# vineetbansal/scarlet

Hardware: AMD Instinct MI355X
Metric: PGM iters/sec on 10k 5-band 64x64 scenes (higher is better)
Workload: dtype f32

## Files before the change

scarlet_amd/csrc/fused2.h:

```cpp
#pragma once
#include "fused.h"

#define SC_FB2 512
#define SC_NW2 (SC_FB2 / SC_WAVE)
#define SC_PAIR_VEC_FLOATS 512

struct KsLengths {
    unsigned short v[2][32];
    static constexpr int fast_len(int n)
    {
        for (int m = n;; ++m) {
            int q = m;
            while (q % 2 == 0) q /= 2;
            while (q % 3 == 0) q /= 3;
            while (q % 5 == 0) q /= 5;
            if (q == 1) return m;
        }
    }
    constexpr KsLengths() : v{}
    {
        for (int r = 0; r < 32; ++r) {
            const int F = fast_len(2 * (2 * r + 1) + 10);
            int Fe = F;
            while (Fe & 1) Fe = fast_len(Fe + 1);
            v[0][r] = (unsigned short)F; v[1][r] = (unsigned short)Fe;
        }
    }
};
__device__ const KsLengths sc_ks_lengths = KsLengths();
__device__ __forceinline__ unsigned ks_request_lengths(int tid)
{
    return tid < 64 ? (unsigned)(&sc_ks_lengths.v[0][0])[tid] : 0u;
}
__device__ __forceinline__ void ks_fill_lengths(unsigned short (*fl)[32], int tid, unsigned requested)
{
    if (tid < 64) (&fl[0][0])[tid] = (unsigned short)requested;
}
__device__ __forceinline__ KsGeom ks_geom(const SymWindow &s, const unsigned short (*fl)[32])
{
    KsGeom g;
    g.h = s.h; g.w = s.w; g.ry = s.h / 2; g.rx = s.w / 2;
    g.ntr = round16(s.h) >> 4; g.wp = round16(s.w); g.ntc = g.wp >> 4;
    g.Fy = uniform((int)fl[0][g.ry]);
    g.Fx = uniform((int)fl[1][g.rx]);
    return g;
}

template <int KM, int BM, int XS, bool P>
__device__ __forceinline__ int iterate2_body(const FusedArgs &a, const int s, const int c0, const int it_old, const bool resident,
                                             const bool reentered = false)
{
    static_assert(KM <= 4, "one pair of waves per component");
    static_assert(1 + KM * BM <= 32 && 4 * SC_NW2 == 32, "the partial sums are combined by 32 rows of 16 lanes");
    constexpr bool X = XS > 0;
    extern __shared__ __align__(16) float lds[];
    const int K = X ? KM : a.K, B = X ? BM : a.B, H = X ? XS : a.H, W = X ? XS : a.W, HW = H * W, LW = X ? SC_XS_STRIDE : tile_stride(W);
    const int tile_floats = H * LW;
#ifndef SC_TILE_B128
#define SC_TILE_B128 1
#endif
    auto tl4 = [](const float *p) {
        if constexpr (X && SC_TILE_B128 && (SC_XS_STRIDE % 4) == 0) return *reinterpret_cast<const float4 *>(p);
        else return lds_load4(p);
    };
    auto ts4 = [](float *p, float4 v) {
        if constexpr (X && SC_TILE_B128 && (SC_XS_STRIDE % 4) == 0) *reinterpret_cast<float4 *>(p) = v;
        else lds_store4(p, v);
    };
    const bool symmetric = X ? true : a.symmetric != 0, monotonic = X ? true : a.monotonic != 0;
    float *tiles = lds;
    float *vecs = lds + (size_t)K * tile_floats;
    constexpr int NG = KM * (KM + 1) / 2;
    constexpr int NP = 1 + KM * BM;
    constexpr int GPT = 2;
    constexpr int GPW = 8;
    __shared__ float red[4 * SC_NW2][NP > NG ? NP : NG];
    __shared__ double mat[2][KM * KM > BM * BM ? KM * KM : BM * BM];
    __shared__ float sed_s[KM * BM], sed_new[KM * BM];
    __shared__ float step_s[2];
    __shared__ double conv_s[KM][2], conv_m[KM][2][2];
    __shared__ int lstop_s[KM];
    __shared__ float nmax_s[KM][2];
    __shared__ int pair_flag[KM][2];
    __shared__ double cent_s[KM][2][3];
    __shared__ unsigned short fl_s[2][32];
    __shared__ int ctl_s[2][2];
    __shared__ int carry_cen[KM][2];
    __shared__ double carry_sh[KM][2];
    __shared__ float carry_sed[KM * BM];
    __shared__ short rowrange_s[KM][2][2];
    const int tid = threadIdx.x, lane = tid & 63, wid = uniform(tid >> 6);
    float *const morph0 = a.morph[0], *const morph1 = a.morph[1], *const sed0 = a.sed[0], *const sed1 = a.sed[1];
    const float *min_g = (c0 ? morph1 : morph0) + (size_t)s * K * HW;
    float *mout_g = (c0 ? morph0 : morph1) + (size_t)s * K * HW;
    const float *sed_in = (c0 ? sed1 : sed0) + (size_t)s * K * B;
    float *sed_out = (c0 ? sed0 : sed1) + (size_t)s * K * B;
    const int it_new = it_old + 1;
    const int ngroups = HW >> 2, gpr = W >> 2;
    const float *img = a.images + (size_t)s * B * HW;
    const float *wgt = (!X && a.weights) ? a.weights + (size_t)s * B * HW : nullptr;
#define STAMP(i) do { if (a.stamps && tid == 0) a.stamps[(size_t)s * 16 + (i)] = (long long)__builtin_amdgcn_s_memtime(); } while (0)
    STAMP(0);
    if (a.stamps && tid == 0) a.stamps[(size_t)s * 16 + 7] = (long long)__builtin_amdgcn_s_memrealtime();
#ifdef SC_STAMP_PERIOD
    if (P && a.stamps && tid == 0) a.stamps[(size_t)a.S * 16 + (size_t)s * 2 + (it_new & 1)] = (long long)__builtin_amdgcn_s_memrealtime();
#endif
    if (P && a.stamps && tid == 0 && !reentered) {
        a.stamps[(size_t)s * 16 + 14] = (long long)__builtin_amdgcn_s_memrealtime();
        a.stamps[(size_t)s * 16 + 15] = (long long)__builtin_amdgcn_s_getreg(4 | (0 << 6) | (31 << 11))
                                        | ((long long)__builtin_amdgcn_s_getreg(20 | (0 << 6) | (31 << 11)) << 32);
    }
    const unsigned fl_req = ks_request_lengths(tid);
    int pre_cy = 0, pre_cx = 0;
    double pre_dy = 0, pre_dx = 0;
    if (X && (wid >> 1) < K) {
        const int cpre = s * K + (wid >> 1);
        if (!(P && reentered)) {
            pre_cy = a.centers[2 * cpre]; pre_cx = a.centers[2 * cpre + 1];
            pre_dy = a.shifts[2 * cpre]; pre_dx = a.shifts[2 * cpre + 1];
        }
        if (P) {
            const int lcy = carry_cen[wid >> 1][0], lcx = carry_cen[wid >> 1][1];
            const double ldy = carry_sh[wid >> 1][0], ldx = carry_sh[wid >> 1][1];
            if (reentered) { pre_cy = lcy; pre_cx = lcx; pre_dy = ldy; pre_dx = ldx; }
        }
    }
    float *kcache = nullptr;
    float kc_v[3] = {0.f, 0.f, 0.f};
    unsigned kc_hdr = 0;
    if (X && a.kscache && (wid >> 1) < K) {
        kcache = a.kscache + ((size_t)(s * K + (wid >> 1)) * 2 + (wid & 1)) * SC_KSC_FLOATS;
        if (P) {
            kc_v[0] = __builtin_nontemporal_load(kcache + lane); kc_v[1] = __builtin_nontemporal_load(kcache + 64 + lane);
            kc_v[2] = __builtin_nontemporal_load(kcache + 128 + lane);
            kc_hdr = __builtin_nontemporal_load(reinterpret_cast<const unsigned *>(kcache) + 192 + (lane & 7));
        } else {
            kc_v[0] = kcache[lane]; kc_v[1] = kcache[64 + lane]; kc_v[2] = kcache[128 + lane];
            kc_hdr = reinterpret_cast<const unsigned *>(kcache)[192 + (lane & 7)];
        }
    }

    float4 mreg[GPT][KM];
    auto load4 = [&](const float *p, bool past_l1) {
        if (P && past_l1) {
            const f32x4 v = __builtin_nontemporal_load(reinterpret_cast<const f32x4 *>(p));
            return make_float4(v[0], v[1], v[2], v[3]);
        }
        return *reinterpret_cast<const float4 *>(p);
    };
    if (!P || !resident) {
#pragma unroll
        for (int j = 0; j < GPT; ++j) {
            const int g = tid + j * SC_FB2;
#pragma unroll
            for (int k = 0; k < KM; ++k)
                mreg[j][k] = (g < ngroups && k < K) ? load4(min_g + (size_t)k * HW + 4 * (size_t)g, reentered)
                                                   : make_float4(0.f, 0.f, 0.f, 0.f);
        }
    }
    float4 ireg[GPT][BM];
    auto load_images = [&](int j) {
        const int g = tid + j * SC_FB2;
#pragma unroll
        for (int b = 0; b < BM; ++b)
            ireg[j][b] = (g < ngroups && b < B) ? reinterpret_cast<const float4 *>(img + (size_t)b * HW)[g]
                                               : make_float4(0.f, 0.f, 0.f, 0.f);
    };
    load_images(0);
    for (int i = tid; i < K * B; i += SC_FB2) {
        float v = 0.f;
        if (!(P && reentered)) v = sed_in[i];
        if (P) { const float lv = carry_sed[(i / B) * BM + (i % B)]; if (reentered) v = lv; }
        if (P && !reentered) carry_sed[(i / B) * BM + (i % B)] = v;
        sed_s[(i / B) * BM + (i % B)] = v;
    }
    ks_fill_lengths(fl_s, tid, fl_req);
    if (tid < 2 * KM) (&pair_flag[0][0])[tid] = 0;
    if (P && tid == 0) { ctl_s[it_old & 1][0] = 1; ctl_s[it_old & 1][1] = 1; }
    if (P && !reentered && tid < KM * 4) (&rowrange_s[0][0][0])[tid] = (short)((tid & 1) ? H - 1 : 0);
    if (P && resident) {
#pragma unroll
        for (int j = 0; j < GPT; ++j) {
            const int g = tid + j * SC_FB2;
            const int y = g / gpr, x = (g - y * gpr) << 2;
#pragma unroll
            for (int k = 0; k < KM; ++k)
                mreg[j][k] = (g < ngroups && k < K) ? tl4(tiles + k * tile_floats + y * LW + x) : make_float4(0.f, 0.f, 0.f, 0.f);
        }
    }
    const bool small_side = (K <= B);
    __syncthreads();
    {
        f32x2 gram2[NG];
#pragma unroll
        for (int i = 0; i < NG; ++i) gram2[i] = (f32x2){0.f, 0.f};
#pragma unroll
        for (int j = 0; j < GPT; ++j) {
            const int g = tid + j * SC_FB2;
            if (g < ngroups) {
                const int y = g / gpr, x = (g - y * gpr) << 2;
#pragma unroll
                for (int k = 0; k < KM; ++k)
                    if (k < K && !(P && resident)) ts4(tiles + k * tile_floats + y * LW + x, mreg[j][k]);
                int gi = 0;
#pragma unroll
                for (int k = 0; k < KM; ++k)
#pragma unroll
                    for (int k2 = k; k2 < KM; ++k2) {
                        const float4 p = mreg[j][k], q = mreg[j][k2];
                        gram2[gi] += (f32x2){p.x, p.y} * (f32x2){q.x, q.y};
                        gram2[gi] += (f32x2){p.z, p.w} * (f32x2){q.z, q.w};
                        ++gi;
                    }
            }
        }
        float gram[NG];
#pragma unroll
        for (int i = 0; i < NG; ++i) gram[i] = gram2[i].x + gram2[i].y;
        float gq[(NG + 3) / 4];
        wave_rowsum_quads(gram, gq);
        if ((lane & 12) == 12) {
#pragma unroll
            for (int m = 0; m < (NG + 3) / 4; ++m)
                if (4 * m + 3 < NG || 4 * m + (lane & 3) < NG) red[4 * wid + (lane >> 4)][4 * m + (lane & 3)] = gq[m];
        }
    }
#pragma unroll
    for (int j = 1; j < GPT; ++j) load_images(j);
    __syncthreads();
    STAMP(1);
    if (wid == 0) {
        {
            const int e = lane >> 2, q = lane & 3;
            const int k = e / K, k2 = e - k * K;
            const int lo = k < k2 ? k : k2, hi = k < k2 ? k2 : k;
            const int go = lo * KM - (lo * (lo - 1)) / 2 + (hi - lo);
            double r = 0;
            if (e < K * K) {
#pragma unroll
                for (int w = 0; w < SC_NW2; ++w) r += (double)red[q * SC_NW2 + w][go];
            }
            r += dpp_mov<SC_DPP_XOR1>(r);
            r += dpp_mov<SC_DPP_XOR2>(r);
            if (e < K * K && q == 0) mat[0][k * KM + k2] = r;
        }
        if (lane < (small_side ? K * K : B * B)) {
            double r = 0;
            if (small_side) {
                const int k = lane / K, k2 = lane - k * K;
                for (int b = 0; b < B; ++b) r += (double)sed_s[k * BM + b] * sed_s[k2 * BM + b];
                mat[1][k * KM + k2] = r;
            } else {
                const int b = lane / B, b2 = lane - b * B;
                for (int k = 0; k < K; ++k) r += (double)sed_s[k * BM + b] * sed_s[k * BM + b2];
                mat[1][b * BM + b2] = r;
            }
        }
        wave_sync();
        if (lane < 2) {
            const int n = (lane == 0 || small_side) ? K : B, ld = (lane == 0 || small_side) ? KM : BM;
            const double L = n <= 4 ? lambda_max_charpoly4(mat[lane], n, ld) : jacobi_lambda_max(mat[lane], n, ld);
            step_s[lane] = 1.0f / (float)L;
            a.lipschitz[2 * s + lane] = L;
        }
    }
    __syncthreads();
    STAMP(2);
    const float step_sed = step_s[0], step_morph = step_s[1];

    {
        float sed[KM][BM];
#pragma unroll
        for (int k = 0; k < KM; ++k)
#pragma unroll
            for (int b = 0; b < BM; ++b)
                sed[k][b] = (k < K && b < B) ? __builtin_bit_cast(float, __builtin_amdgcn_readfirstlane(
                                                   __builtin_bit_cast(int, sed_s[k * BM + b]))) : 0.f;
        bool fixm[KM];
#pragma unroll
        for (int k = 0; k < KM; ++k) fixm[k] = (k < K) && a.fix_morph && a.fix_morph[(size_t)s * K + k];
        f32x2 dsed2[KM][BM];
#pragma unroll
        for (int k = 0; k < KM; ++k)
#pragma unroll
            for (int b = 0; b < BM; ++b) dsed2[k][b] = (f32x2){0.f, 0.f};
        f32x2 loss2 = {0.f, 0.f};
        const f32x2 ws2 = {a.weight_scalar, a.weight_scalar};
#pragma unroll
        for (int j = 0; j < GPT; ++j) {
            const int g = tid + j * SC_FB2;
            if (g < ngroups) {
                const int y = g / gpr, x = (g - y * gpr) << 2;
                f32x2 m2[KM][2], gm2[KM][2];
#pragma unroll
                for (int k = 0; k < KM; ++k) {
                    float4 v = make_float4(0.f, 0.f, 0.f, 0.f);
                    if (k < K) v = tl4(tiles + k * tile_floats + y * LW + x);
                    m2[k][0] = (f32x2){v.x, v.y}; m2[k][1] = (f32x2){v.z, v.w};
                    gm2[k][0] = (f32x2){0.f, 0.f}; gm2[k][1] = gm2[k][0];
                }
#pragma unroll
                for (int b = 0; b < BM; ++b) {
                    if (b < B) {
                        const float4 iv = ireg[j][b];
                        f32x2 im2[2] = {{iv.x, iv.y}, {iv.z, iv.w}}, ww2[2] = {ws2, ws2};
                        if (wgt) {
                            const float4 wv = reinterpret_cast<const float4 *>(wgt + (size_t)b * HW)[g];
                            ww2[0] = (f32x2){wv.x, wv.y}; ww2[1] = (f32x2){wv.z, wv.w};
                        }
#pragma unroll
                        for (int p = 0; p < 2; ++p) {
                            f32x2 model = sed[0][b] * m2[0][p];
#pragma unroll
                            for (int k = 1; k < KM; ++k) model += sed[k][b] * m2[k][p];
                            const f32x2 d = X ? model - im2[p] : ww2[p] * (model - im2[p]);
                            loss2 = (f32x2){__builtin_fmaf(d.x, d.x, loss2.x), __builtin_fmaf(d.y, d.y, loss2.y)};
                            const f32x2 gg = X ? d : ww2[p] * d;
#pragma unroll
                            for (int k = 0; k < KM; ++k) { dsed2[k][b] += gg * m2[k][p]; gm2[k][p] += sed[k][b] * gg; }
                        }
                    }
                }
#pragma unroll
                for (int k = 0; k < KM; ++k)
                    if (k < K && !fixm[k]) {
                        const f32x2 o0 = m2[k][0] - step_morph * gm2[k][0], o1 = m2[k][1] - step_morph * gm2[k][1];
                        ts4(tiles + k * tile_floats + y * LW + x, make_float4(o0.x, o0.y, o1.x, o1.y));
                    }
            }
        }
        float part[NP];
        part[0] = 0.5f * (loss2.x + loss2.y);
#pragma unroll
        for (int k = 0; k < KM; ++k)
#pragma unroll
            for (int b = 0; b < BM; ++b) part[1 + k * BM + b] = dsed2[k][b].x + dsed2[k][b].y;
        float pq[(NP + 3) / 4];
        wave_rowsum_quads(part, pq);
        if ((lane & 12) == 12) {
#pragma unroll
            for (int m = 0; m < (NP + 3) / 4; ++m)
                if (4 * m + 3 < NP || 4 * m + (lane & 3) < NP) red[4 * wid + (lane >> 4)][4 * m + (lane & 3)] = pq[m];
        }
    }
    __syncthreads();
    STAMP(3);
    {
        const int i = tid >> 4, p = tid & 15;
        const bool live = i < 1 + K * B;
        const int src = (!live || i == 0) ? 0 : 1 + ((i - 1) / B) * BM + (i - 1) % B;
        double r = live ? (double)red[p][src] + (double)red[p + 16][src] : 0.0;
        r += dpp_mov<SC_DPP_XOR1>(r);
        r += dpp_mov<SC_DPP_XOR2>(r);
        r += dpp_mov<SC_DPP_HALF_MIRROR>(r);
        r += dpp_mov<SC_DPP_MIRROR>(r);
        if (live && p == 0) {
            if (i == 0) {
                if (it_new <= a.mse_capacity) a.mse[(size_t)s * a.mse_capacity + it_new - 1] = r;
            } else {
                const int k = (i - 1) / B, b = (i - 1) - k * B;
                const float curv = sed_s[k * BM + b];
                const bool fixed = a.fix_sed && a.fix_sed[(size_t)s * K + k];
                sed_new[k * BM + b] = fixed ? curv : curv - step_sed * (float)r;
            }
        }
    }
    __syncthreads();
    STAMP(4);

    const int k = wid >> 1, half = wid & 1;
    const bool lead = half == ((k >> 1) & 1);
    auto pair_sync = [&](int phase, auto long_wait) {
        constexpr bool LONG = decltype(long_wait)::value;
        __builtin_amdgcn_fence(__ATOMIC_RELEASE, "workgroup");
        if (lane == 0) __hip_atomic_store(&pair_flag[k & (KM - 1)][half], phase, __ATOMIC_RELAXED, __HIP_MEMORY_SCOPE_WORKGROUP);
        while (__hip_atomic_load(&pair_flag[k & (KM - 1)][1 - half], __ATOMIC_RELAXED, __HIP_MEMORY_SCOPE_WORKGROUP) < phase) {
            if (LONG) __builtin_amdgcn_s_sleep(8); else __builtin_amdgcn_s_sleep(2);
        }
        __builtin_amdgcn_fence(__ATOMIC_ACQUIRE, "workgroup");
    };
    const int n_present = a.ncomp ? scene_ncomp(a.ncomp, s, K) : K;
    const bool mine = k < n_present;
    const int c = s * K + (mine ? k : 0);
    Tile t; t.H = H; t.W = W; t.LW = LW; t.m = tiles + (mine ? k : 0) * tile_floats;
    float *vec = vecs + (mine ? k : 0) * SC_PAIR_VEC_FLOATS;
    float *zv = vec + 384 + SC_WAVE * half;
    int cy = 0, cx = 0, stat = 0;
    int mode = 0;
    SymWindow sw = {0, 0, 1, 1, true};
    KsGeom kg = {};
    float sy = 0.f;
    bool rank1 = false;
    if (mine) {
        cy = X ? pre_cy : a.centers[2 * c]; cx = X ? pre_cx : a.centers[2 * c + 1];
        wave_max_pixel(t, cy, cx, stat);
        cy = uniform(cy); cx = uniform(cx);
        if (symmetric) {
            double dy = X ? pre_dy : a.shifts[2 * c], dx = X ? pre_dx : a.shifts[2 * c + 1];
            if (it_new % 5 == 0) {
                double p0, p1, p2;
                wave_centroid_sums(t, a.centroid_psf, a.centroid_P, cy, cx, half, 2, p0, p1, p2);
                if (lane == 0) { cent_s[k][half][0] = p0; cent_s[k][half][1] = p1; cent_s[k][half][2] = p2; }
                pair_sync(1, std::false_type{});
                wave_centroid_finish(t, a.centroid_P, cent_s[k][0][0] + cent_s[k][1][0], cent_s[k][0][1] + cent_s[k][1][1],
                                     cent_s[k][0][2] + cent_s[k][1][2], cy, cx, dy, dx, stat);
                if (lead && lane == 0) { a.shifts[2 * c] = dy; a.shifts[2 * c + 1] = dx; }
            }
            cy = uniform(cy); cx = uniform(cx); dy = uniform(dy); dx = uniform(dx);
            if (P && lead && lane == 0) { carry_cen[k][0] = cy; carry_cen[k][1] = cx; carry_sh[k][0] = dy; carry_sh[k][1] = dx; }
            sw = sym_window(H, W, cy, cx);
            mode = (dy != dy) ? 2 : (sw.centered ? 0 : 1);
            if (mode == 1) {
                kg = ks_geom(sw, fl_s);
                const unsigned key[6] = {(unsigned)H << 24 | (unsigned)W << 16 | (unsigned)cy << 8 | (unsigned)cx, SC_KSC_MAGIC,
                                         (unsigned)__double2loint(dy), (unsigned)__double2hiint(dy),
                                         (unsigned)__double2loint(dx), (unsigned)__double2hiint(dx)};
                bool hit = kcache != nullptr;
#pragma unroll
                for (int i = 0; i < 6; ++i) hit = hit && (unsigned)__builtin_amdgcn_readlane((int)kc_hdr, i) == key[i];
                if (hit) {
                    const int q = lane + SC_WAVE * half;
                    vec[q] = kc_v[0]; vec[128 + q] = kc_v[1]; vec[256 + q] = kc_v[2];
                    sy = __int_as_float(__builtin_amdgcn_readlane((int)kc_hdr, 6));
                } else {
                    sy = pair_ks_vectors(kg, dy, dx, vec, half, kc_v);
                    if (kcache) {
                        kcache[lane] = kc_v[0]; kcache[64 + lane] = kc_v[1]; kcache[128 + lane] = kc_v[2];
                        unsigned word = __float_as_uint(sy);
#pragma unroll
                        for (int i = 0; i < 6; ++i) word = lane == i ? key[i] : word;
                        if (lane < 7) reinterpret_cast<unsigned *>(kcache)[192 + lane] = word;
                    }
                }
                rank1 = sy != 0.f;
                if (rank1) pair_ks_colsums(t, sw, kg, zv);
            }
        }
    }
    STAMP(8);
    if (mine) pair_sync(2, std::false_type{});
    STAMP(12);
    f32x4 T[4][2];
    if (mine && mode == 1) {
        if (rank1) pair_ks_z(kg, vec + 256, zv);
        pair_ks_gemm1<true>(t, sw, kg, vec, half, T);
    }
    if (mine) pair_sync(3, std::false_type{});
    STAMP(13);
    if (mine && mode == 1) pair_ks_gemm2<true>(t, sw, kg, vec, zv, half, T, sy, rank1);
    if (mine && mode == 2 && lead) wave_flip_symmetry<float>(t, sw, false, 1.0f);
    if (mine) pair_sync(4, std::false_type{});
    STAMP(9);
    const int dyq = (2 * SC_WAVE) / gpr, dxq = 2 * SC_WAVE - dyq * gpr;
    const int g0 = lane + SC_WAVE * half;
    const int y0 = g0 / gpr, x0 = g0 - y0 * gpr;
    int rl_lo = 0, rl_hi = H - 1, ro_lo = 0, ro_hi = H - 1;
    if (P && mine) {
        rl_lo = uniform((int)rowrange_s[k][c0][0]); rl_hi = uniform((int)rowrange_s[k][c0][1]);
        ro_lo = uniform((int)rowrange_s[k][1 - c0][0]); ro_hi = uniform((int)rowrange_s[k][1 - c0][1]);
    }
    float4 lastv[GPW];
    auto load_last = [&]() {
        const float4 *last4 = reinterpret_cast<const float4 *>(min_g + (size_t)k * HW);
#pragma unroll
        for (int j = 0; j < GPW; ++j) {
            const int g = g0 + j * 2 * SC_WAVE;
            const int row = y0 + j * dyq;
            const bool want = g < ngroups && (!P || (row >= rl_lo && row <= rl_hi));
            lastv[j] = want ? load4(reinterpret_cast<const float *>(last4 + g), true) : make_float4(0.f, 0.f, 0.f, 0.f);
        }
    };
    if (mine && !lead) load_last();
    if (mine && lead) {
        int lstop = 1 << 30;
        if (monotonic) wave_monotonic<float>(t, cy, cx, 0.f, &lstop);
        if (lane == 0) {
            lstop_s[k] = lstop; a.centers[2 * c] = cy; a.centers[2 * c + 1] = cx;
            if (P) nmax_s[k][0] = t.m[cy * LW + cx];
        }
        load_last();
    }
    if (mine) pair_sync(5, std::true_type{});
    STAMP(10);
    float norm = 0.f;
    float l0 = (!X && a.l0_thresh >= 0.f) ? a.l0_thresh * step_morph : -1.f;
    float l1 = (!X && a.l1_thresh >= 0.f) ? a.l1_thresh * step_morph : -1.f;
    auto sparse = [&](float v) {
        if (l0 >= 0.f && fabsf(v) < l0) v = 0.f;
        if (l1 >= 0.f) {
            const float mag = fabsf(v) - l1;
            v = (v > 0.f ? 1.f : (v < 0.f ? -1.f : 0.f)) * (mag < 0.f ? 0.f : mag);
        }
        return v;
    };
    if (!monotonic) {
        float vmax = -INFINITY;
        bool anynan = false;
        if (mine) {
            int y = y0, xq = x0;
            for (int g = g0; g < ngroups; g += 2 * SC_WAVE) {
                float *p = t.m + y * LW + (xq << 2);
                float4 v = lds_load4(p);
                v.x = sparse(v.x); v.y = sparse(v.y); v.z = sparse(v.z); v.w = sparse(v.w);
                v.x = v.x < 0.f ? 0.f : v.x; v.y = v.y < 0.f ? 0.f : v.y;
                v.z = v.z < 0.f ? 0.f : v.z; v.w = v.w < 0.f ? 0.f : v.w;
                anynan |= (v.x != v.x) | (v.y != v.y) | (v.z != v.z) | (v.w != v.w);
                vmax = fmaxf(fmaxf(vmax, fmaxf(v.x, v.y)), fmaxf(v.z, v.w));
                lds_store4(p, v);
                y += dyq; xq += dxq;
                if (xq >= gpr) { xq -= gpr; ++y; }
            }
            vmax = wave_max(vmax);
            if (__any(anynan)) vmax = __builtin_nanf("");
            if (lane == 0) nmax_s[k][half] = vmax;
        }
        if (mine) pair_sync(6, std::false_type{});
        if (mine) {
            const float m0 = nmax_s[k][0], m1 = nmax_s[k][1];
            norm = (m0 != m0 || m1 != m1) ? __builtin_nanf("") : fmaxf(m0, m1);
        }
        l0 = -1.f; l1 = -1.f;
    } else if (mine) {
        norm = sparse(P ? nmax_s[k][0] : t.m[cy * LW + cx]);
        if (norm < 0.f) norm = 0.f;
    }
    if (mine) {
        const int lstop = lstop_s[k];
        const bool cut = lstop < (1 << 30);
        const bool regular = norm > 0.f && !isinf(norm);
        const float rnorm = 1.0f / norm;
        float4 *out4 = reinterpret_cast<float4 *>(mout_g + (size_t)k * HW);
        f32x2 d2p = {0.f, 0.f}, n2p = {0.f, 0.f};
        const f32x2 rn2 = {rnorm, rnorm}, nm2 = {norm, norm};
        int u_lo = 0, u_hi = H - 1;
        if (P && cut && regular && l0 < 0.f && l1 < 0.f) {
            const int rt = lstop >> 1;
            u_lo = min(min(rl_lo, ro_lo), max(cy - rt, 0)); u_hi = max(max(rl_hi, ro_hi), min(cy + rt, H - 1));
        }
        auto final_pass = [&](auto cut_c, auto gen_c) {
            constexpr bool CUT = decltype(cut_c)::value, GEN = decltype(gen_c)::value;
            int y = y0, xq = x0;
#pragma unroll
            for (int j = 0; j < GPW; ++j) {
                const int g = g0 + j * 2 * SC_WAVE;
                const int yw = uniform(y0 + j * dyq) & ~3;
                const bool skip = P && X && (yw + 3 < u_lo || yw > u_hi);
                if (g < ngroups && skip) ts4(t.m + y * LW + (xq << 2), make_float4(0.f, 0.f, 0.f, 0.f));
                if (g < ngroups && !skip) {
                    const float4 v4 = tl4(t.m + y * LW + (xq << 2));
                    const float4 l = lastv[j];
                    float v[4] = {v4.x, v4.y, v4.z, v4.w};
                    int axmax = 0, xb = 0;
                    if (CUT) {
                        const int ay = y < cy ? cy - y : y - cy;
                        const int h1 = (lstop - ay) >> 1;
                        axmax = h1 >= ay ? h1 : lstop - 2 * ay;
                        xb = (xq << 2) - cx + axmax;
                    }
#pragma unroll
                    for (int e = 0; e < 4; ++e) {
                        if (GEN) v[e] = sparse(v[e]);
                        const bool beyond = CUT && (axmax < 0 || (unsigned)(xb + e) > (unsigned)(2 * axmax));
                        v[e] = (v[e] < 0.f || beyond) ? 0.f : v[e];
                    }
                    f32x2 o01, o23;
                    if (GEN && !regular) {
                        o01 = (f32x2){v[0] / norm, v[1] / norm}; o23 = (f32x2){v[2] / norm, v[3] / norm};
                    } else {
                        const f32x2 a01 = {v[0], v[1]}, a23 = {v[2], v[3]};
                        const f32x2 q01 = a01 * rn2, q23 = a23 * rn2;
                        o01 = (a01 - q01 * nm2) * rn2 + q01;
                        o23 = (a23 - q23 * nm2) * rn2 + q23;
                    }
                    const float4 o4 = make_float4(o01.x, o01.y, o23.x, o23.y);
                    out4[g] = o4;
                    if (P) ts4(t.m + y * LW + (xq << 2), o4);
                    const f32x2 e01 = (f32x2){l.x, l.y} - o01, e23 = (f32x2){l.z, l.w} - o23;
                    d2p += e01 * e01; d2p += e23 * e23;
                    n2p += o01 * o01; n2p += o23 * o23;
                }
                y += dyq; xq += dxq;
                if (xq >= gpr) { xq -= gpr; ++y; }
                if (j & 1) __builtin_amdgcn_sched_barrier(0);
            }
        };
        using std::true_type; using std::false_type;
        if (regular && l0 < 0.f && l1 < 0.f) {
            if (cut) final_pass(true_type{}, false_type{}); else final_pass(false_type{}, false_type{});
        } else {
            final_pass(true_type{}, true_type{});
        }
        const double d2 = wave_sum((double)(d2p.x + d2p.y)), n2 = wave_sum((double)(n2p.x + n2p.y));
        if (lane == 0) { conv_m[k][half][0] = d2; conv_m[k][half][1] = n2; }
        if (P && lead && lane == 0) {
            const bool known = cut && regular && l0 < 0.f && l1 < 0.f;
            rowrange_s[k][1 - c0][0] = (short)(known ? max(cy - (lstop >> 1), 0) : 0);
            rowrange_s[k][1 - c0][1] = (short)(known ? min(cy + (lstop >> 1), H - 1) : H - 1);
        }
        if (lead) {
            double d2s = 0, n2s = 0;
            if (lane < B) {
                float v = sed_new[k * BM + lane];
                if (v < 0.f) v = 0.f;
                v = v * norm;
                sed_out[k * B + lane] = v;
                if (P) carry_sed[k * BM + lane] = v;
                const float d = sed_s[k * BM + lane] - v;
                d2s = (double)(d * d);
                n2s = (double)(v * v);
            }
            d2s = wave_sum(d2s); n2s = wave_sum(n2s);
            if (lane == 0) { conv_s[k][0] = d2s; conv_s[k][1] = n2s; }
        }
    }
    __syncthreads();
    if (mine && norm == norm) {
        const double n2 = conv_m[k][0][1] + conv_m[k][1][1];
        if (n2 != n2) {
            norm = __builtin_nanf("");
            float4 *out4 = reinterpret_cast<float4 *>(mout_g + (size_t)k * HW);
            const float4 nan4 = make_float4(norm, norm, norm, norm);
            for (int g = g0; g < ngroups; g += 2 * SC_WAVE) out4[g] = nan4;
            if (lead && lane < B) { sed_out[k * B + lane] = norm; if (P) carry_sed[k * BM + lane] = norm; }
            if (P && lane == 0) {
                ctl_s[it_old & 1][1] = 0;
                rowrange_s[k][1 - c0][0] = 0; rowrange_s[k][1 - c0][1] = (short)(H - 1);
            }
        }
    }
    if (mine && lead && lane == 0) {
        if (!(norm > 0.f) || isinf(norm)) stat |= SCARLET_STATUS_NONFINITE;
        if (stat) atomicOr(&a.status[s], stat);
    }
    STAMP(5);

    if (wid == 0) {
        bool pending = false;
        if (lane < n_present && it_new > 1) {
            const int kk = lane;
            int set = 0;
            const double d2 = conv_m[kk][0][0] + conv_m[kk][1][0], n2 = conv_m[kk][0][1] + conv_m[kk][1][1];
            if (!(n2 == n2 && conv_s[kk][0] <= a.e_rel2 * conv_s[kk][1])) set |= SCARLET_FLAG_SED_NOT_CONVERGED;
            if (!(d2 <= a.e_rel2 * n2)) set |= SCARLET_FLAG_MORPH_NOT_CONVERGED;
            const int clear = (SCARLET_FLAG_SED_NOT_CONVERGED | SCARLET_FLAG_MORPH_NOT_CONVERGED) & ~set;
            if (clear) atomicAnd(&a.flags[s * K + kk], ~clear);
            if (set) atomicOr(&a.flags[s * K + kk], set);
            pending = set != 0;
        }
        const bool done = it_new > 1 && __builtin_amdgcn_ballot_w64(pending) == 0;
        if (lane == 0) {
            a.it[s] = it_new;
            a.cur[s] = 1 - c0;
            if (done) { a.active[s] = 0; if (P) ctl_s[it_old & 1][0] = 0; }
        }
    }
    STAMP(6);
    if (a.stamps && tid == 0) a.stamps[(size_t)s * 16 + 11] = (long long)__builtin_amdgcn_s_memrealtime();
#undef STAMP
    if (P) {
        __syncthreads();
        return uniform(ctl_s[it_old & 1][0] | (ctl_s[it_old & 1][1] << 1));
    }
    return 0;
}

template <int KM, int BM, int XS = 0>
__global__ __launch_bounds__(SC_FB2, 4) void k_iterate2(FusedArgs a)
{
    const int s = blockIdx.x;
    const int active_s = a.active[s], c0 = a.cur[s], it_old = a.it[s];
    asm volatile("" ::"s"(c0), "s"(it_old));
    if (!active_s) return;
    iterate2_body<KM, BM, XS, false>(a, s, c0, it_old, false);
}

#define SC_FIT2X_KERNEL k_fit2x
#define SC_FIT2X_REENTER(scene, state, it)                                                                     \
    asm volatile("s_mov_b64 exec, -1\n\t"                                                                      \
                 "s_mov_b64 s[0:1], %0\n\t"                                                                    \
                 "s_mov_b32 s2, %1\n\t"                                                                        \
                 "s_mov_b32 s3, %2\n\t"                                                                        \
                 "s_mov_b32 s4, %3\n\t"                                                                        \
                 "v_mov_b32 v0, %4\n\t"                                                                        \
                 "s_getpc_b64 s[6:7]\n\t"                                                                      \
                 "s_add_u32 s6, s6, k_fit2x@rel32@lo+4\n\t"                                                    \
                 "s_addc_u32 s7, s7, k_fit2x@rel32@hi+12\n\t"                                                  \
                 "s_waitcnt lgkmcnt(0)\n\t"                                                                    \
                 "s_setpc_b64 s[6:7]"                                                                          \
                 :                                                                                             \
                 : "s"(__builtin_amdgcn_kernarg_segment_ptr()), "s"(scene), "s"(state), "s"(it), "v"((int)threadIdx.x) \
                 : "s0", "s1", "s2", "s3", "s4", "s6", "s7", "v0", "scc", "memory")
extern "C" __global__ __launch_bounds__(SC_FB2, 4) void SC_FIT2X_KERNEL(FusedArgs a, int n_iter, int *queue, int n_workgroups)
{
    const int s = blockIdx.x;
    const unsigned st = (unsigned)__builtin_amdgcn_workgroup_id_y();
    int c0 = 0, it = 0, left = 0;
    bool resident = false, run = true;
    if (st >> 31) {
        resident = ((st >> 30) & 1) && !(n_iter & (1 << 30));
        c0 = (int)((st >> 29) & 1); left = (int)(st & 0x1fffffffu);
        it = (int)__builtin_amdgcn_workgroup_id_z();
    } else {
        const int active_s = a.active[s];
        c0 = a.cur[s]; it = a.it[s];
        asm volatile("" ::"s"(c0), "s"(it));
        left = n_iter & 0xffffff;
        run = active_s && left > 0;
    }
    if (run) {
        const int r = iterate2_body<4, 5, 64, true>(a, s, c0, it, resident, (st >> 31) != 0);
        if ((r & 1) && left > 1) {
            const unsigned nst = 0x80000000u | ((unsigned)(r >> 1) << 30) | ((unsigned)(c0 ^ 1) << 29) | (unsigned)(left - 1);
            if (!(r & 2) || (n_iter & (1 << 30))) {
                asm volatile("s_waitcnt vmcnt(0)" ::: "memory");
                __syncthreads();
            }
            SC_FIT2X_REENTER(s, nst, it + 1);
        }
    }
    __shared__ int next_s;
    if (threadIdx.x == 0) next_s = queue ? atomicAdd(queue, 1) + n_workgroups : a.S;
    __syncthreads();
    const int nx = uniform(next_s);
    __syncthreads();
    if (nx < a.S) SC_FIT2X_REENTER(nx, 0u, 0);
}
```

scarlet_amd/csrc/common.h:

```cpp
#pragma once
#include <hip/hip_runtime.h>
#include <stdint.h>
#include "../../include/scarlet_hip.h"

#define SC_WAVE 64
#define SC_BLOCK 256
#define SC_NWAVES (SC_BLOCK / SC_WAVE)

typedef float f32x4 __attribute__((ext_vector_type(4)));

template <int CTRL>
__device__ __forceinline__ float dpp_mov(float v) {
    return __int_as_float(__builtin_amdgcn_update_dpp(0, __float_as_int(v), CTRL, 0xf, 0xf, true));
}
template <int CTRL>
__device__ __forceinline__ double dpp_mov(double v) {
    const int lo = __builtin_amdgcn_update_dpp(0, __double2loint(v), CTRL, 0xf, 0xf, true);
    const int hi = __builtin_amdgcn_update_dpp(0, __double2hiint(v), CTRL, 0xf, 0xf, true);
    return __hiloint2double(hi, lo);
}
__device__ __forceinline__ float read_lane(float v, int lane) {
    return __int_as_float(__builtin_amdgcn_readlane(__float_as_int(v), lane));
}
__device__ __forceinline__ double read_lane(double v, int lane) {
    return __hiloint2double(__builtin_amdgcn_readlane(__double2hiint(v), lane),
                            __builtin_amdgcn_readlane(__double2loint(v), lane));
}
__device__ __forceinline__ int uniform(int v) { return __builtin_amdgcn_readfirstlane(v); }
__device__ __forceinline__ double uniform(double v) {
    return __hiloint2double(__builtin_amdgcn_readfirstlane(__double2hiint(v)),
                            __builtin_amdgcn_readfirstlane(__double2loint(v)));
}
__device__ __forceinline__ int scene_ncomp(const int *ncomp, int s, int K)
{
    if (!ncomp) return K;
    const int n = ncomp[s];
    return (n >= 1 && n <= K) ? n : 0;
}
#define SC_DPP_XOR1 0xB1
#define SC_DPP_XOR2 0x4E
#define SC_DPP_HALF_MIRROR 0x141
#define SC_DPP_MIRROR 0x140
template <typename T>
__device__ __forceinline__ T wave_sum(T v) {
    v += dpp_mov<SC_DPP_XOR1>(v);
    v += dpp_mov<SC_DPP_XOR2>(v);
    v += dpp_mov<SC_DPP_HALF_MIRROR>(v);
    v += dpp_mov<SC_DPP_MIRROR>(v);
    return (read_lane(v, 0) + read_lane(v, 16)) + (read_lane(v, 32) + read_lane(v, 48));
}
__device__ __forceinline__ float wave_max(float v) {
    v = fmaxf(v, dpp_mov<SC_DPP_XOR1>(v));
    v = fmaxf(v, dpp_mov<SC_DPP_XOR2>(v));
    v = fmaxf(v, dpp_mov<SC_DPP_HALF_MIRROR>(v));
    v = fmaxf(v, dpp_mov<SC_DPP_MIRROR>(v));
    return fmaxf(fmaxf(read_lane(v, 0), read_lane(v, 16)), fmaxf(read_lane(v, 32), read_lane(v, 48)));
}

#define SC_DPP_BCAST15 0x142
#define SC_DPP_BCAST31 0x143
template <int N>
__device__ __forceinline__ void wave_sum_lastrow(float (&v)[N]) {
#pragma unroll
    for (int i = 0; i < N; ++i) v[i] += dpp_mov<SC_DPP_XOR1>(v[i]);
#pragma unroll
    for (int i = 0; i < N; ++i) v[i] += dpp_mov<SC_DPP_XOR2>(v[i]);
#pragma unroll
    for (int i = 0; i < N; ++i) v[i] += dpp_mov<SC_DPP_HALF_MIRROR>(v[i]);
#pragma unroll
    for (int i = 0; i < N; ++i) v[i] += dpp_mov<SC_DPP_MIRROR>(v[i]);
#pragma unroll
    for (int i = 0; i < N; ++i)
        v[i] += __int_as_float(__builtin_amdgcn_update_dpp(0, __float_as_int(v[i]), SC_DPP_BCAST15, 0xa, 0xf, false));
#pragma unroll
    for (int i = 0; i < N; ++i)
        v[i] += __int_as_float(__builtin_amdgcn_update_dpp(0, __float_as_int(v[i]), SC_DPP_BCAST31, 0xc, 0xf, false));
}

#define SC_DPP_ROR4 0x124
#define SC_DPP_ROR8 0x128
template <int N>
__device__ __forceinline__ void wave_rowsum_quads(const float (&v)[N], float (&out)[(N + 3) / 4]) {
    constexpr int N2 = (N + 1) / 2, N4 = (N + 3) / 4;
    const int lane = threadIdx.x & (SC_WAVE - 1);
    const bool b0 = lane & 1, b1 = lane & 2;
    float r[N2];
#pragma unroll
    for (int i = 0; i < N2; ++i) {
        const float a = v[2 * i] + dpp_mov<SC_DPP_XOR1>(v[2 * i]);
        if (2 * i + 1 < N) {
            const float b = v[2 * i + 1] + dpp_mov<SC_DPP_XOR1>(v[2 * i + 1]);
            r[i] = b0 ? b : a;
        } else r[i] = a;
    }
#pragma unroll
    for (int i = 0; i < N4; ++i) {
        const float a = r[2 * i] + dpp_mov<SC_DPP_XOR2>(r[2 * i]);
        if (2 * i + 1 < N2) {
            const float b = r[2 * i + 1] + dpp_mov<SC_DPP_XOR2>(r[2 * i + 1]);
            out[i] = b1 ? b : a;
        } else out[i] = a;
    }
#pragma unroll
    for (int i = 0; i < N4; ++i) out[i] += dpp_mov<SC_DPP_ROR4>(out[i]);
#pragma unroll
    for (int i = 0; i < N4; ++i) out[i] += dpp_mov<SC_DPP_ROR8>(out[i]);
}

__device__ __forceinline__ double block_sum(double v, double *red) {
    v = wave_sum(v);
    const int lane = threadIdx.x & (SC_WAVE - 1), wid = threadIdx.x / SC_WAVE;
    __syncthreads();
    if (lane == 0) red[wid] = v;
    __syncthreads();
    double r = 0;
#pragma unroll
    for (int w = 0; w < SC_NWAVES; ++w) r += red[w];
    return r;
}
__device__ __forceinline__ float block_max_nan(float v, bool isnan_any, float *red) {
    v = wave_max(v);
    unsigned long long nanmask = __ballot(isnan_any);
    const int lane = threadIdx.x & (SC_WAVE - 1), wid = threadIdx.x / SC_WAVE;
    __syncthreads();
    if (lane == 0) red[wid] = nanmask ? __builtin_nanf("") : v;
    __syncthreads();
    float r = red[0];
    bool bad = r != r;
#pragma unroll
    for (int w = 1; w < SC_NWAVES; ++w) { float t = red[w]; bad |= (t != t); r = fmaxf(r, t); }
    return bad ? __builtin_nanf("") : r;
}

__device__ __forceinline__ void lds_store4(float *p, float4 v)
{
    reinterpret_cast<float2 *>(p)[0] = make_float2(v.x, v.y);
    reinterpret_cast<float2 *>(p)[1] = make_float2(v.z, v.w);
}
__device__ __forceinline__ float4 lds_load4(const float *p)
{
    const float2 a = reinterpret_cast<const float2 *>(p)[0], b = reinterpret_cast<const float2 *>(p)[1];
    return make_float4(a.x, a.y, b.x, b.y);
}

#define SC_NFL_MAX 2304
#define SC_RANK1_COLS ((SCARLET_MAX_SIDE + SC_BLOCK - 1) / SC_BLOCK)
extern __constant__ unsigned short sc_nfl_table[SC_NFL_MAX];

__device__ __forceinline__ int dev_next_fast_len(int n) { return sc_nfl_table[n]; }

__host__ __device__ __forceinline__ int tile_stride(int W) { return ((W - 2 + 31) / 32) * 32 + 2; }
#ifndef SC_XS_STRIDE
#define SC_XS_STRIDE 68
#endif
__host__ __device__ __forceinline__ int scratch_stride(int wp) { return ((wp + 31) / 32) * 32 + 16; }
__host__ __device__ __forceinline__ int round16(int v) { return (v + 15) & ~15; }
```

Before: 15.94 million.

## Overlap Lipschitz solves and SED update with morphology work via flag sync

Moves the SED-side Lipschitz solve and the SED gradient update off the critical path. Wave 1 now computes them while the morph waves proceed, and signals completion through an LDS flag with release/acquire fences in place of a full barrier. The morph-step Lipschitz for the next iteration is computed at the end of the current one from the carried SED and reused on resident re-entry. Image loads are hoisted to the start and Gram partials are parked in the vector region. This adds a spin-wait and relies on the carried state being valid when resident.

```diff
diff --git a/scarlet_amd/csrc/fused2.h b/scarlet_amd/csrc/fused2.h
--- a/scarlet_amd/csrc/fused2.h
+++ b/scarlet_amd/csrc/fused2.h
@@ -48,7 +48,7 @@
 
 template <int KM, int BM, int XS, bool P>
 __device__ __forceinline__ int iterate2_body(const FusedArgs &a, const int s, const int c0, const int it_old, const bool resident,
-                                             const bool reentered = false)
+                                             const bool reentered = false, const bool carried = false)
 {
     static_assert(KM <= 4, "one pair of waves per component");
     static_assert(1 + KM * BM <= 32 && 4 * SC_NW2 == 32, "the partial sums are combined by 32 rows of 16 lanes");
@@ -74,10 +74,13 @@
     constexpr int NP = 1 + KM * BM;
     constexpr int GPT = 2;
     constexpr int GPW = 8;
+    static_assert(4 * SC_NW2 * NG <= SC_PAIR_VEC_FLOATS, "the Gram partials are parked in one pair's vector region");
     __shared__ float red[4 * SC_NW2][NP > NG ? NP : NG];
+    float (*const gred)[NG] = reinterpret_cast<float (*)[NG]>(vecs);
     __shared__ double mat[2][KM * KM > BM * BM ? KM * KM : BM * BM];
     __shared__ float sed_s[KM * BM], sed_new[KM * BM];
-    __shared__ float step_s[2];
+    __shared__ float step_morph_s;
+    __shared__ int sed_flag;
     __shared__ double conv_s[KM][2], conv_m[KM][2][2];
     __shared__ int lstop_s[KM];
     __shared__ float nmax_s[KM][2];
@@ -166,7 +169,8 @@
             ireg[j][b] = (g < ngroups && b < B) ? reinterpret_cast<const float4 *>(img + (size_t)b * HW)[g]
                                                : make_float4(0.f, 0.f, 0.f, 0.f);
     };
-    load_images(0);
+#pragma unroll
+    for (int j = 0; j < GPT; ++j) load_images(j);
     for (int i = tid; i < K * B; i += SC_FB2) {
         float v = 0.f;
         if (!(P && reentered)) v = sed_in[i];
@@ -176,6 +180,7 @@
     }
     ks_fill_lengths(fl_s, tid, fl_req);
     if (tid < 2 * KM) (&pair_flag[0][0])[tid] = 0;
+    if (tid == 2 * KM) sed_flag = 0;
     if (P && tid == 0) { ctl_s[it_old & 1][0] = 1; ctl_s[it_old & 1][1] = 1; }
     if (P && !reentered && tid < KM * 4) (&rowrange_s[0][0][0])[tid] = (short)((tid & 1) ? H - 1 : 0);
     if (P && resident) {
@@ -222,51 +227,57 @@
         if ((lane & 12) == 12) {
 #pragma unroll
             for (int m = 0; m < (NG + 3) / 4; ++m)
-                if (4 * m + 3 < NG || 4 * m + (lane & 3) < NG) red[4 * wid + (lane >> 4)][4 * m + (lane & 3)] = gq[m];
-        }
-    }
-#pragma unroll
-    for (int j = 1; j < GPT; ++j) load_images(j);
-    __syncthreads();
-    STAMP(1);
-    if (wid == 0) {
-        {
-            const int e = lane >> 2, q = lane & 3;
-            const int k = e / K, k2 = e - k * K;
-            const int lo = k < k2 ? k : k2, hi = k < k2 ? k2 : k;
-            const int go = lo * KM - (lo * (lo - 1)) / 2 + (hi - lo);
-            double r = 0;
-            if (e < K * K) {
-#pragma unroll
-                for (int w = 0; w < SC_NW2; ++w) r += (double)red[q * SC_NW2 + w][go];
-            }
-            r += dpp_mov<SC_DPP_XOR1>(r);
-            r += dpp_mov<SC_DPP_XOR2>(r);
-            if (e < K * K && q == 0) mat[0][k * KM + k2] = r;
-        }
+                if (4 * m + 3 < NG || 4 * m + (lane & 3) < NG) gred[4 * wid + (lane >> 4)][4 * m + (lane & 3)] = gq[m];
+        }
+    }
+    auto sed_gram = [&](const float *sd) {
         if (lane < (small_side ? K * K : B * B)) {
             double r = 0;
             if (small_side) {
                 const int k = lane / K, k2 = lane - k * K;
-                for (int b = 0; b < B; ++b) r += (double)sed_s[k * BM + b] * sed_s[k2 * BM + b];
+                for (int b = 0; b < B; ++b) r += (double)sd[k * BM + b] * sd[k2 * BM + b];
                 mat[1][k * KM + k2] = r;
             } else {
                 const int b = lane / B, b2 = lane - b * B;
-                for (int k = 0; k < K; ++k) r += (double)sed_s[k * BM + b] * sed_s[k * BM + b2];
+                for (int k = 0; k < K; ++k) r += (double)sd[k * BM + b] * sd[k * BM + b2];
                 mat[1][b * BM + b2] = r;
             }
         }
         wave_sync();
-        if (lane < 2) {
-            const int n = (lane == 0 || small_side) ? K : B, ld = (lane == 0 || small_side) ? KM : BM;
-            const double L = n <= 4 ? lambda_max_charpoly4(mat[lane], n, ld) : jacobi_lambda_max(mat[lane], n, ld);
-            step_s[lane] = 1.0f / (float)L;
-            a.lipschitz[2 * s + lane] = L;
+    };
+    auto solve = [&](const double *M, int n, int ld) {
+        return n <= 4 ? lambda_max_charpoly4(M, n, ld) : jacobi_lambda_max(const_cast<double *>(M), n, ld);
+    };
+    if (wid == 0) {
+        if (P && carried) {
+            if (lane == 0) a.lipschitz[2 * s + 1] = mat[1][0];
+        } else {
+            sed_gram(sed_s);
+            if (lane == 0) {
+                const double L = solve(mat[1], small_side ? K : B, small_side ? KM : BM);
+                step_morph_s = 1.0f / (float)L;
+                a.lipschitz[2 * s + 1] = L;
+            }
         }
     }
     __syncthreads();
+    STAMP(1);
+    if (wid == 1) {
+        const int e = lane >> 2, q = lane & 3;
+        const int k = e / K, k2 = e - k * K;
+        const int lo = k < k2 ? k : k2, hi = k < k2 ? k2 : k;
+        const int go = lo * KM - (lo * (lo - 1)) / 2 + (hi - lo);
+        double r = 0;
+        if (e < K * K) {
+#pragma unroll
+            for (int w = 0; w < SC_NW2; ++w) r += (double)gred[q * SC_NW2 + w][go];
+        }
+        r += dpp_mov<SC_DPP_XOR1>(r);
+        r += dpp_mov<SC_DPP_XOR2>(r);
+        if (e < K * K && q == 0) mat[0][k * KM + k2] = r;
+    }
     STAMP(2);
-    const float step_sed = step_s[0], step_morph = step_s[1];
+    const float step_morph = step_morph_s;
 
     {
         float sed[KM][BM];
@@ -345,27 +356,6 @@
     }
     __syncthreads();
     STAMP(3);
-    {
-        const int i = tid >> 4, p = tid & 15;
-        const bool live = i < 1 + K * B;
-        const int src = (!live || i == 0) ? 0 : 1 + ((i - 1) / B) * BM + (i - 1) % B;
-        double r = live ? (double)red[p][src] + (double)red[p + 16][src] : 0.0;
-        r += dpp_mov<SC_DPP_XOR1>(r);
-        r += dpp_mov<SC_DPP_XOR2>(r);
-        r += dpp_mov<SC_DPP_HALF_MIRROR>(r);
-        r += dpp_mov<SC_DPP_MIRROR>(r);
-        if (live && p == 0) {
-            if (i == 0) {
-                if (it_new <= a.mse_capacity) a.mse[(size_t)s * a.mse_capacity + it_new - 1] = r;
-            } else {
-                const int k = (i - 1) / B, b = (i - 1) - k * B;
-                const float curv = sed_s[k * BM + b];
-                const bool fixed = a.fix_sed && a.fix_sed[(size_t)s * K + k];
-                sed_new[k * BM + b] = fixed ? curv : curv - step_sed * (float)r;
-            }
-        }
-    }
-    __syncthreads();
     STAMP(4);
 
     const int k = wid >> 1, half = wid & 1;
@@ -480,6 +470,38 @@
         }
         load_last();
     }
+    if (wid == 1) {
+        float step_sed = 0.f;
+        if (lane == 0) {
+            const double L = solve(mat[0], K, KM);
+            step_sed = 1.0f / (float)L;
+            a.lipschitz[2 * s] = L;
+        }
+        step_sed = read_lane(step_sed, 0);
+#pragma unroll 1
+        for (int i0 = 0; i0 < 1 + K * B; i0 += 4) {
+            const int i = i0 + (lane >> 4), p = lane & 15;
+            const bool live = i < 1 + K * B;
+            const int src = (!live || i == 0) ? 0 : 1 + ((i - 1) / B) * BM + (i - 1) % B;
+            double r = live ? (double)red[p][src] + (double)red[p + 16][src] : 0.0;
+            r += dpp_mov<SC_DPP_XOR1>(r);
+            r += dpp_mov<SC_DPP_XOR2>(r);
+            r += dpp_mov<SC_DPP_HALF_MIRROR>(r);
+            r += dpp_mov<SC_DPP_MIRROR>(r);
+            if (live && p == 0) {
+                if (i == 0) {
+                    if (it_new <= a.mse_capacity) a.mse[(size_t)s * a.mse_capacity + it_new - 1] = r;
+                } else {
+                    const int kk = (i - 1) / B, b = (i - 1) - kk * B;
+                    const float curv = sed_s[kk * BM + b];
+                    const bool fixed = a.fix_sed && a.fix_sed[(size_t)s * K + kk];
+                    sed_new[kk * BM + b] = fixed ? curv : curv - step_sed * (float)r;
+                }
+            }
+        }
+        __builtin_amdgcn_fence(__ATOMIC_RELEASE, "workgroup");
+        if (lane == 0) __hip_atomic_store(&sed_flag, 1, __ATOMIC_RELAXED, __HIP_MEMORY_SCOPE_WORKGROUP);
+    }
     if (mine) pair_sync(5, std::true_type{});
     STAMP(10);
     float norm = 0.f;
@@ -598,6 +620,8 @@
             rowrange_s[k][1 - c0][1] = (short)(known ? min(cy + (lstop >> 1), H - 1) : H - 1);
         }
         if (lead) {
+            while (__hip_atomic_load(&sed_flag, __ATOMIC_RELAXED, __HIP_MEMORY_SCOPE_WORKGROUP) == 0) __builtin_amdgcn_s_sleep(2);
+            __builtin_amdgcn_fence(__ATOMIC_ACQUIRE, "workgroup");
             double d2s = 0, n2s = 0;
             if (lane < B) {
                 float v = sed_new[k * BM + lane];
@@ -634,6 +658,14 @@
     }
     STAMP(5);
 
+    if (P && wid == 1) {
+        sed_gram(carry_sed);
+        if (lane == 0) {
+            const double L = solve(mat[1], small_side ? K : B, small_side ? KM : BM);
+            step_morph_s = 1.0f / (float)L;
+            mat[1][0] = L;
+        }
+    }
     if (wid == 0) {
         bool pending = false;
         if (lane < n_present && it_new > 1) {
@@ -708,7 +740,7 @@
         run = active_s && left > 0;
     }
     if (run) {
-        const int r = iterate2_body<4, 5, 64, true>(a, s, c0, it, resident, (st >> 31) != 0);
+        const int r = iterate2_body<4, 5, 64, true>(a, s, c0, it, resident, (st >> 31) != 0, (st >> 30) == 3u);
         if ((r & 1) && left > 1) {
             const unsigned nst = 0x80000000u | ((unsigned)(r >> 1) << 30) | ((unsigned)(c0 ^ 1) << 29) | (unsigned)(left - 1);
             if (!(r & 2) || (n_iter & (1 << 30))) {
```

New measurement: 15.91 million. About the same (-0.2%).

## Move monotonic SED update and Lipschitz estimation onto idle non-lead waves

Applied to the files above, without the earlier changes.

In the monotonic path the SED gradient step, its normalisation and convergence sums, and the morph Lipschitz eigenvalue solve move off the serial lead-wave path. The last non-lead wave to arrive, counted with a workgroup atomic, does this work while the lead waves run the monotonic projection. In persistent mode that wave also precomputes the next iteration's SED Gram matrix and step, so re-entered resident scenes skip recomputing it. This adds an atomic arrival counter and more cross-wave shared-memory dependencies, which brings ordering risk.

```diff
diff --git a/scarlet_amd/csrc/common.h b/scarlet_amd/csrc/common.h
--- a/scarlet_amd/csrc/common.h
+++ b/scarlet_amd/csrc/common.h
@@ -48,6 +48,14 @@
     v += dpp_mov<SC_DPP_HALF_MIRROR>(v);
     v += dpp_mov<SC_DPP_MIRROR>(v);
     return (read_lane(v, 0) + read_lane(v, 16)) + (read_lane(v, 32) + read_lane(v, 48));
+}
+template <typename T>
+__device__ __forceinline__ T row_sum(T v) {
+    v += dpp_mov<SC_DPP_XOR1>(v);
+    v += dpp_mov<SC_DPP_XOR2>(v);
+    v += dpp_mov<SC_DPP_HALF_MIRROR>(v);
+    v += dpp_mov<SC_DPP_MIRROR>(v);
+    return v;
 }
 __device__ __forceinline__ float wave_max(float v) {
     v = fmaxf(v, dpp_mov<SC_DPP_XOR1>(v));
diff --git a/scarlet_amd/csrc/fused2.h b/scarlet_amd/csrc/fused2.h
--- a/scarlet_amd/csrc/fused2.h
+++ b/scarlet_amd/csrc/fused2.h
@@ -82,6 +82,7 @@
     __shared__ int lstop_s[KM];
     __shared__ float nmax_s[KM][2];
     __shared__ int pair_flag[KM][2];
+    __shared__ int arrive_s;
     __shared__ double cent_s[KM][2][3];
     __shared__ unsigned short fl_s[2][32];
     __shared__ int ctl_s[2][2];
@@ -100,6 +101,11 @@
     const float *img = a.images + (size_t)s * B * HW;
     const float *wgt = (!X && a.weights) ? a.weights + (size_t)s * B * HW : nullptr;
 #define STAMP(i) do { if (a.stamps && tid == 0) a.stamps[(size_t)s * 16 + (i)] = (long long)__builtin_amdgcn_s_memtime(); } while (0)
+#ifdef SC_STAMP_WORKER
+#define WSTAMP(i) do { if (a.stamps && lane == 0) a.stamps[(size_t)s * 16 + 12 + (i)] = (long long)__builtin_amdgcn_s_memtime(); } while (0)
+#else
+#define WSTAMP(i) do { } while (0)
+#endif
     STAMP(0);
     if (a.stamps && tid == 0) a.stamps[(size_t)s * 16 + 7] = (long long)__builtin_amdgcn_s_memrealtime();
 #ifdef SC_STAMP_PERIOD
@@ -176,6 +182,7 @@
     }
     ks_fill_lengths(fl_s, tid, fl_req);
     if (tid < 2 * KM) (&pair_flag[0][0])[tid] = 0;
+    if (tid == 2 * KM) arrive_s = 0;
     if (P && tid == 0) { ctl_s[it_old & 1][0] = 1; ctl_s[it_old & 1][1] = 1; }
     if (P && !reentered && tid < KM * 4) (&rowrange_s[0][0][0])[tid] = (short)((tid & 1) ? H - 1 : 0);
     if (P && resident) {
@@ -189,6 +196,20 @@
         }
     }
     const bool small_side = (K <= B);
+    const int n_present = a.ncomp ? scene_ncomp(a.ncomp, s, K) : K;
+    const bool carried = P && reentered && resident && monotonic && n_present > 0;
+    auto sed_gram = [&](const float *sed, double *m) {
+        double r = 0;
+        if (small_side) {
+            const int k = lane / K, k2 = lane - k * K;
+            for (int b = 0; b < B; ++b) r += (double)sed[k * BM + b] * sed[k2 * BM + b];
+            m[k * KM + k2] = r;
+        } else {
+            const int b = lane / B, b2 = lane - b * B;
+            for (int k = 0; k < K; ++k) r += (double)sed[k * BM + b] * sed[k * BM + b2];
+            m[b * BM + b2] = r;
+        }
+    };
     __syncthreads();
     {
         f32x2 gram2[NG];
@@ -244,24 +265,17 @@
             r += dpp_mov<SC_DPP_XOR2>(r);
             if (e < K * K && q == 0) mat[0][k * KM + k2] = r;
         }
-        if (lane < (small_side ? K * K : B * B)) {
-            double r = 0;
-            if (small_side) {
-                const int k = lane / K, k2 = lane - k * K;
-                for (int b = 0; b < B; ++b) r += (double)sed_s[k * BM + b] * sed_s[k2 * BM + b];
-                mat[1][k * KM + k2] = r;
-            } else {
-                const int b = lane / B, b2 = lane - b * B;
-                for (int k = 0; k < K; ++k) r += (double)sed_s[k * BM + b] * sed_s[k * BM + b2];
-                mat[1][b * BM + b2] = r;
-            }
-        }
-        wave_sync();
-        if (lane < 2) {
-            const int n = (lane == 0 || small_side) ? K : B, ld = (lane == 0 || small_side) ? KM : BM;
-            const double L = n <= 4 ? lambda_max_charpoly4(mat[lane], n, ld) : jacobi_lambda_max(mat[lane], n, ld);
-            step_s[lane] = 1.0f / (float)L;
-            a.lipschitz[2 * s + lane] = L;
+        if (carried) {
+            if (lane == 1) a.lipschitz[2 * s + 1] = mat[1][0];
+        } else {
+            if (lane < (small_side ? K * K : B * B)) sed_gram(sed_s, mat[1]);
+            wave_sync();
+            if (lane < 2 && !(monotonic && lane == 0)) {
+                const int n = (lane == 0 || small_side) ? K : B, ld = (lane == 0 || small_side) ? KM : BM;
+                const double L = n <= 4 ? lambda_max_charpoly4(mat[lane], n, ld) : jacobi_lambda_max(mat[lane], n, ld);
+                step_s[lane] = 1.0f / (float)L;
+                a.lipschitz[2 * s + lane] = L;
+            }
         }
     }
     __syncthreads();
@@ -359,9 +373,13 @@
                 if (it_new <= a.mse_capacity) a.mse[(size_t)s * a.mse_capacity + it_new - 1] = r;
             } else {
                 const int k = (i - 1) / B, b = (i - 1) - k * B;
-                const float curv = sed_s[k * BM + b];
-                const bool fixed = a.fix_sed && a.fix_sed[(size_t)s * K + k];
-                sed_new[k * BM + b] = fixed ? curv : curv - step_sed * (float)r;
+                if (monotonic) {
+                    sed_new[k * BM + b] = (float)r;
+                } else {
+                    const float curv = sed_s[k * BM + b];
+                    const bool fixed = a.fix_sed && a.fix_sed[(size_t)s * K + k];
+                    sed_new[k * BM + b] = fixed ? curv : curv - step_sed * (float)r;
+                }
             }
         }
     }
@@ -379,7 +397,6 @@
         }
         __builtin_amdgcn_fence(__ATOMIC_ACQUIRE, "workgroup");
     };
-    const int n_present = a.ncomp ? scene_ncomp(a.ncomp, s, K) : K;
     const bool mine = k < n_present;
     const int c = s * K + (mine ? k : 0);
     Tile t; t.H = H; t.W = W; t.LW = LW; t.m = tiles + (mine ? k : 0) * tile_floats;
@@ -439,14 +456,18 @@
     }
     STAMP(8);
     if (mine) pair_sync(2, std::false_type{});
+#ifndef SC_STAMP_WORKER
     STAMP(12);
+#endif
     f32x4 T[4][2];
     if (mine && mode == 1) {
         if (rank1) pair_ks_z(kg, vec + 256, zv);
         pair_ks_gemm1<true>(t, sw, kg, vec, half, T);
     }
     if (mine) pair_sync(3, std::false_type{});
+#ifndef SC_STAMP_WORKER
     STAMP(13);
+#endif
     if (mine && mode == 1) pair_ks_gemm2<true>(t, sw, kg, vec, zv, half, T, sy, rank1);
     if (mine && mode == 2 && lead) wave_flip_symmetry<float>(t, sw, false, 1.0f);
     if (mine) pair_sync(4, std::false_type{});
@@ -470,19 +491,6 @@
             lastv[j] = want ? load4(reinterpret_cast<const float *>(last4 + g), true) : make_float4(0.f, 0.f, 0.f, 0.f);
         }
     };
-    if (mine && !lead) load_last();
-    if (mine && lead) {
-        int lstop = 1 << 30;
-        if (monotonic) wave_monotonic<float>(t, cy, cx, 0.f, &lstop);
-        if (lane == 0) {
-            lstop_s[k] = lstop; a.centers[2 * c] = cy; a.centers[2 * c + 1] = cx;
-            if (P) nmax_s[k][0] = t.m[cy * LW + cx];
-        }
-        load_last();
-    }
-    if (mine) pair_sync(5, std::true_type{});
-    STAMP(10);
-    float norm = 0.f;
     float l0 = (!X && a.l0_thresh >= 0.f) ? a.l0_thresh * step_morph : -1.f;
     float l1 = (!X && a.l1_thresh >= 0.f) ? a.l1_thresh * step_morph : -1.f;
     auto sparse = [&](float v) {
@@ -493,6 +501,67 @@
         }
         return v;
     };
+    if (mine && !lead) load_last();
+    if (monotonic && mine && !lead) {
+        float peak = sparse(t.m[cy * LW + cx]);
+        if (peak < 0.f) peak = 0.f;
+        int arrived = 0;
+        if (lane == 0) nmax_s[k][1] = peak;
+        __builtin_amdgcn_fence(__ATOMIC_RELEASE, "workgroup");
+        if (lane == 0) arrived = __hip_atomic_fetch_add(&arrive_s, 1, __ATOMIC_RELAXED, __HIP_MEMORY_SCOPE_WORKGROUP);
+        if (uniform(arrived) == n_present - 1) {
+            __builtin_amdgcn_fence(__ATOMIC_ACQUIRE, "workgroup");
+            WSTAMP(0);
+            float step_w = 0.f;
+            if (lane == 0) {
+                const double L = lambda_max_charpoly4(mat[0], K, KM);
+                a.lipschitz[2 * s] = L;
+                step_w = 1.0f / (float)L;
+            }
+            step_w = read_lane(step_w, 0);
+            const int kk = lane >> 4, bb = lane & 15;
+            const bool entry = kk < n_present && bb < B;
+            double d2s = 0, n2s = 0;
+            if (entry) {
+                const float curv = sed_s[kk * BM + bb];
+                const bool fixed = a.fix_sed && a.fix_sed[(size_t)s * K + kk];
+                float v = fixed ? curv : curv - step_w * sed_new[kk * BM + bb];
+                if (v < 0.f) v = 0.f;
+                v = v * nmax_s[kk][1];
+                sed_out[kk * B + bb] = v;
+                if (P) carry_sed[kk * BM + bb] = v;
+                const float d = curv - v;
+                d2s = (double)(d * d);
+                n2s = (double)(v * v);
+            }
+            d2s = row_sum(d2s); n2s = row_sum(n2s);
+            if (entry && bb == 0) { conv_s[kk][0] = d2s; conv_s[kk][1] = n2s; }
+            if (P) {
+                wave_sync();
+                if (lane < (small_side ? K * K : B * B)) sed_gram(carry_sed, mat[1]);
+                wave_sync();
+                if (lane == 0) {
+                    const int n = small_side ? K : B, ld = small_side ? KM : BM;
+                    const double L = n <= 4 ? lambda_max_charpoly4(mat[1], n, ld) : jacobi_lambda_max(mat[1], n, ld);
+                    step_s[1] = 1.0f / (float)L;
+                    mat[1][0] = L;
+                }
+            }
+            WSTAMP(1);
+        }
+    }
+    if (mine && lead) {
+        int lstop = 1 << 30;
+        if (monotonic) wave_monotonic<float>(t, cy, cx, 0.f, &lstop);
+        if (lane == 0) {
+            lstop_s[k] = lstop; a.centers[2 * c] = cy; a.centers[2 * c + 1] = cx;
+            if (P) nmax_s[k][0] = t.m[cy * LW + cx];
+        }
+        load_last();
+    }
+    if (mine) pair_sync(5, std::true_type{});
+    STAMP(10);
+    float norm = 0.f;
     if (!monotonic) {
         float vmax = -INFINITY;
         bool anynan = false;
@@ -597,7 +666,7 @@
             rowrange_s[k][1 - c0][0] = (short)(known ? max(cy - (lstop >> 1), 0) : 0);
             rowrange_s[k][1 - c0][1] = (short)(known ? min(cy + (lstop >> 1), H - 1) : H - 1);
         }
-        if (lead) {
+        if (lead && !monotonic) {
             double d2s = 0, n2s = 0;
             if (lane < B) {
                 float v = sed_new[k * BM + lane];
@@ -657,6 +726,7 @@
     STAMP(6);
     if (a.stamps && tid == 0) a.stamps[(size_t)s * 16 + 11] = (long long)__builtin_amdgcn_s_memrealtime();
 #undef STAMP
+#undef WSTAMP
     if (P) {
         __syncthreads();
         return uniform(ctl_s[it_old & 1][0] | (ctl_s[it_old & 1][1] << 1));
```

Result: faster. 15.85 million before, 16.16 million after (median of 6 runs) (+2.0%).
